# flo-stilz/Audio-Key-Estimation

Measured on AMD Instinct MI355X. Metric: clips/s (15 s @ 22.05 kHz), HIP CQT + PitchClassNet forward, higher is better.
Workload: dtype f32 accumulation everywhere; pitch / semitone / layer-0 convolutions: f16 activations x f16 weights (per-channel power-of-two scaled) on MFMA, one product; last layer's pitch-class convolutions and heads: 3-term split-bf16 on MFMA (hi*hi + lo*hi + hi*lo); CQT filter bank: 3-term split-bf16 on MFMA

## Files before the change

### audio-key-estimation_amd/csrc/pcnet.hip

```cpp
#include <algorithm>
#include <cmath>
#include <cstdlib>
#include <cstring>
#include <map>
#include <string>
#include <vector>

#include "common.h"
#include "pcnet_kernels.h"
#include "pcnet_bwd_kernels.h"

using namespace ake_k;

namespace {

constexpr double kBnEps = 1e-5;
constexpr size_t kLdsBudget = 64 * 1024;
constexpr size_t kBfFragsPerConv = 14 * 2 * 64 + 64;

struct TensorSpec {
    std::string name;
    int64_t shape[4];
    int ndim;
};
// ... 1699 lines not shown
}

int upload_i32(const std::vector<int32_t>& v, int32_t** dev) {
    if (*dev) { (void)hipFree(*dev); *dev = nullptr; }
    AKE_HIP_CHECK(hipMalloc(dev, std::max<size_t>(v.size(), 1) * sizeof(int32_t)));
    AKE_HIP_CHECK(hipMemcpy(*dev, v.data(), v.size() * sizeof(int32_t), hipMemcpyHostToDevice));
    return AKE_OK;
}

int rebuild_dense_affine(ake_pcnet* n, const float* params_dev, hipStream_t s) {
    if (n->aff_recs.empty()) return AKE_OK;
    const int rows = static_cast<int>(n->dense_aff_floats / 3);
    if (!n->dense_aff_dev) {
        std::vector<int32_t> idx;
        idx.reserve(static_cast<size_t>(rows) * 5);
        auto off = [&](const std::string& key) { return static_cast<int32_t>(n->grad_off[n->spec_index.at(key)]); };
        for (const auto& r : n->aff_recs)
            for (int ch = 0; ch < r.C; ++ch) {
                int32_t bits;
                std::memcpy(&bits, &r.slope, sizeof(bits));
                for (const char* f : {".weight", ".bias", ".running_mean", ".running_var"}) idx.push_back(off(r.bn + f) + ch);
                idx.push_back(bits);
            }
        int rc = upload_i32(idx, &n->dense_aff_idx_dev);
        if (rc) return rc;
        AKE_HIP_CHECK(hipMalloc(&n->dense_aff_dev, n->dense_aff_floats * sizeof(float)));
    }
    ake::ProfScope ps("dense_affine_kernel", s);
    hipLaunchKernelGGL(dense_affine_kernel, dim3((rows + 255) / 256), dim3(256), 0, s, params_dev, n->dense_aff_idx_dev, n->dense_aff_dev, rows);
    AKE_HIP_CHECK(hipGetLastError());
    return AKE_OK;
}

int build_fold_tables(ake_pcnet* n) {
    std::vector<int32_t> fold_ch(n->grad_floats, -1), fold_bn, run_off(static_cast<size_t>(n->bn_channels) * 2, 0), run_off2(static_cast<size_t>(n->bn_channels) * 2, -1);
    n->recomputed_bn_channels = 0;
    auto off = [&](const std::string& key) { return static_cast<int32_t>(n->grad_off[n->spec_index.at(key)]); };
    int base = 0;
    for (const auto& r : n->fold_records) {
        const int32_t w0 = off(r.wkey), b0 = off(r.bkey);
        const size_t total = r.per_out * r.cout, k = r.transposed ? r.per_out / r.cin : 0;
        for (size_t i = 0; i < total; ++i) {
            const int co = r.transposed ? static_cast<int>((i / k) % r.cout) : static_cast<int>(i / r.per_out);
            fold_ch[w0 + i] = (base + co) << 1;
        }
        for (int co = 0; co < r.cout; ++co) {
            fold_ch[b0 + co] = ((base + co) << 1) | 1;
            fold_bn.push_back(off(r.bn + ".weight") + co);
            fold_bn.push_back(off(r.bn + ".bias") + co);
            fold_bn.push_back(off(r.bn + ".running_mean") + co);
            fold_bn.push_back(off(r.bn + ".running_var") + co);
        }
        base += r.cout;
    }
    for (const auto& l : n->bns)
        for (int c = 0; c < l.C; ++c) {
            run_off[2 * (l.ch_off + c)] = off(l.name + ".running_mean") + c;
            run_off[2 * (l.ch_off + c) + 1] = off(l.name + ".running_var") + c;
            const bool again = n->cfg.denseblock && l.name.size() > 6 && l.name.compare(l.name.size() - 6, 6, ".norm1") == 0;
            if (again) {
                run_off2[2 * (l.ch_off + c)] = run_off[2 * (l.ch_off + c)];
                run_off2[2 * (l.ch_off + c) + 1] = run_off[2 * (l.ch_off + c) + 1];
                ++n->recomputed_bn_channels;
            }
        }
    int rc;
    if ((rc = upload_i32(fold_ch, &n->fold_ch_dev)) || (rc = upload_i32(fold_bn, &n->fold_bn_dev)) || (rc = upload_i32(run_off, &n->run_off_dev)) || (rc = upload_i32(run_off2, &n->run_off2_dev)) ||
        (rc = upload_i32(n->map_host, &n->map_dev)))
        return rc;
    if (n->folded_dev) { (void)hipFree(n->folded_dev); n->folded_dev = nullptr; }
    AKE_HIP_CHECK(hipMalloc(&n->folded_dev, n->grad_floats * sizeof(float)));
    return AKE_OK;
}

bool pc_bf16_eligible(const PackedConv& pc) { return (pc.kh == 12 || pc.kh == 1) && pc.kw == 7 && pc.cin <= 16 && (pc.cout == 16 || pc.cout == 32); }

int rebuild_bf16_frags(ake_pcnet* n, hipStream_t s, bool train_only = false) {
    size_t count = 0;
    for (auto& layer : n->p2p)
        for (size_t j = 0; j < layer.size(); ++j) {
            PackedConv& pc = layer[j];
            pc.bf_off = -1;
            if (pc.cin <= 8 && pc.cout == 8 && pc.kh == 7 && pc.kw == 7 && pc.co == 8) { pc.bf_off = static_cast<long long>(count); count += kBfFragsPerConv; }
        }
    struct TrainFrag { PackedConv* pc; size_t raw; int cin, cout, flip; };
    std::vector<TrainFrag> tfr;
    if (!n->raw_w_off.empty())
        for (size_t i = 1; i < n->p2p_t.size() && i < n->p2p_d.size(); ++i)
            for (size_t j = 0; j < n->p2p_t[i].size() && j < n->p2p_d[i].size(); ++j) {
                PackedConv& pt = n->p2p_t[i][j];
                PackedConv& pd = n->p2p_d[i][j];
                pt.bf_off = pd.bf_off = -1;
                const auto it = n->spec_index.find("model." + std::to_string(i) + ".p2p.layer." + std::to_string(3 * j) + ".weight");
                if (it == n->spec_index.end() || pt.kh != 7 || pt.kw != 7 || pt.cin > 8 || pt.cout > 8 || n->cfg.resblock || n->cfg.denseblock) continue;
                const size_t raw = n->raw_w_off[it->second];
                pt.bf_off = static_cast<long long>(count); count += kBfFragsPerConv;
                tfr.push_back({&pt, raw, pt.cin, pt.cout, 0});
                pd.bf_off = static_cast<long long>(count); count += kBfFragsPerConv;
                tfr.push_back({&pd, raw, pt.cin, pt.cout, 1});
            }
    std::vector<PackedConv*> tpc;
    if (!n->raw_w_off.empty() && !n->cfg.resblock && !n->cfg.denseblock) {
        for (size_t i = 1; i < n->pc2pc_t.size(); ++i)
            for (PackedConv& pc : n->pc2pc_t[i]) tpc.push_back(&pc);
        if (!n->head_key_t.empty()) tpc.push_back(&n->head_key_t[0]);
        if (!n->head_tonic_t.empty()) tpc.push_back(&n->head_tonic_t[0]);
        if (n->head_genre_t.size() == 2) tpc.push_back(&n->head_genre_t[0]);
    }
    for (PackedConv* pc : tpc) {
        pc->bf_off = -1;
        if (pc_bf16_eligible(*pc)) { pc->bf_off = static_cast<long long>(count); count += static_cast<size_t>(pc->kh) * 4 * (pc->cout / 16) * 2 * 64 + 64; }
    }
    std::vector<PackedConv*> tpd;
    if (!n->raw_w_off.empty() && !n->cfg.resblock && !n->cfg.denseblock)
        for (size_t i = 1; i < n->pc2pc_d.size(); ++i)
            for (PackedConv& pc : n->pc2pc_d[i]) tpd.push_back(&pc);
    for (PackedConv* pc : tpd) {
        pc->bf_off = -1;
        if (pc->kh == 12 && pc->kw == 7 && pc->cin == 16 && pc->cout <= 32) {
            pc->bf_off = static_cast<long long>(count);
            count += static_cast<size_t>(pc->kh) * 4 * ((pc->cout + 15) / 16) * 2 * 64 + 64;
        }
    }
    std::vector<PackedConv*> thd;
    if (!n->raw_w_off.empty() && !n->cfg.resblock && !n->cfg.denseblock && n->cfg.head_layers == 2) {
        if (!n->head_key_d.empty()) thd.push_back(&n->head_key_d[0]);
        if (!n->head_tonic_d.empty()) thd.push_back(&n->head_tonic_d[0]);
        if (!n->head_genre_d.empty()) thd.push_back(&n->head_genre_d[0]);
    }
    for (PackedConv* pc : thd) {
        pc->bf_off = pc->bf_off2 = -1;
        if ((pc->kh == 12 || pc->kh == 1) && pc->kw == 7 && pc->cin == 32 && pc->cout == 16) {
            const size_t one = static_cast<size_t>(pc->kh) * 4 * 2 * 64 + 64;
            pc->bf_off = static_cast<long long>(count); pc->bf_off2 = static_cast<long long>(count + one);
            count += 2 * one;
        }
    }
    std::vector<PackedConv*> pcs;
    for (auto& layer : n->pc2pc)
        for (PackedConv& pc : layer) pcs.push_back(&pc);
    if (!n->head_key.empty()) pcs.push_back(&n->head_key[0]);
    if (!n->head_tonic.empty()) pcs.push_back(&n->head_tonic[0]);
    if (n->head_genre.size() == 2) pcs.push_back(&n->head_genre[0]);
    for (PackedConv* pc : pcs) {
        pc->bf_off = -1;
        if (pc_bf16_eligible(*pc)) { pc->bf_off = static_cast<long long>(count); count += static_cast<size_t>(pc->kh) * 4 * (pc->cout / 16) * 2 * 64; }
    }
    std::vector<PackedConv*> h1;
    if (n->head_key.size() == 2) h1.push_back(&n->head_key[1]);
    if (n->head_tonic.size() == 2) h1.push_back(&n->head_tonic[1]);
    if (n->head_genre.size() == 2) h1.push_back(&n->head_genre[1]);
    for (PackedConv* pc : h1) {
        pc->bf_off = -1;
        if ((pc->kh == 12 || pc->kh == 2) && pc->kw == 7 && pc->cout == 1 && pc->co == 1 && pc->cin == 32) { pc->bf_off = static_cast<long long>(count); count += static_cast<size_t>(pc->kh) * 22 * 2 * 64; }
    }
    if (!n->pc2pc.empty())
        for (PackedConv& pc : n->pc2pc[0]) {
            pc.l0_off = -1;
            if (n->cfg.num_layers > 1 && pc.kh == 12 && pc.kw == 7 && pc.co == 4 && pc.groups == 1 && pc.cout <= 4 && pc.cin <= 4) {
                pc.l0_off = static_cast<long long>(count); count += 24 * 64 + 64;
            }
        }
    for (size_t i = 1; i < n->semi.size(); ++i) {
        PackedConv& pc = n->semi[i];
        pc.bf_off = -1;
        if (pc.cin == 8 && pc.co == 8 && pc.groups == 1 && i < n->p2p.size() && !n->p2p[i].empty() && n->p2p[i].back().bf_off >= 0) {
            pc.bf_off = static_cast<long long>(count); count += 6 * 64 + 64;
        }
    }
    if (count == 0) return AKE_OK;
    if (n->bf_frags_count != count) {
        if (n->bf_frags_dev) { (void)hipFree(n->bf_frags_dev); n->bf_frags_dev = nullptr; }
        AKE_HIP_CHECK(hipMalloc(&n->bf_frags_dev, count * sizeof(uint4)));
        n->bf_frags_count = count;
    }
    ake::ProfScope ps("pack_bf16_kernels", s);
    n->eval_frags_stale = train_only;
    if (!train_only)
    for (const auto& layer : n->p2p)
        for (const PackedConv& pc : layer)
            if (pc.bf_off >= 0)
                hipLaunchKernelGGL(pack_p2p_f16_kernel, dim3((14 * 64 + 255) / 256), dim3(256), 0, s, n->blob_dev + pc.w_off, n->bf_frags_dev + pc.bf_off, pc.cin);
    if (!train_only)
    for (const PackedConv* pc : pcs)
        if (pc->bf_off >= 0) {
            const int NT = pc->cout / 16;
            hipLaunchKernelGGL(pack_pc_bf16_kernel, dim3((pc->kh * 4 * NT * 64 + 255) / 256), dim3(256), 0, s, n->blob_dev + pc->w_off,
                               n->bf_frags_dev + pc->bf_off, pc->cin, pc->cout, pc->co, NT, pc->kh);
        }
    if (!train_only && !n->pc2pc.empty())
        for (const PackedConv& pc : n->pc2pc[0])
            if (pc.l0_off >= 0)
                hipLaunchKernelGGL(pack_l0_f16_kernel, dim3(3), dim3(256), 0, s, n->blob_dev + pc.w_off, n->bf_frags_dev + pc.l0_off, pc.cin, pc.cout);
    {
        std::vector<PcPackJob> jobs;
        auto add = [&](const PackedConv* pc, long long off, int NT, int dy_rot, int ci_off) {
            jobs.push_back(PcPackJob{n->blob_dev + pc->w_off, n->bf_frags_dev + off, pc->cin, pc->cout, pc->co, NT, pc->kh, dy_rot, ci_off});
        };
        for (const PackedConv* pc : tpc)
            if (pc->bf_off >= 0) add(pc, pc->bf_off, pc->cout / 16, 0, 0);
        for (const PackedConv* pc : tpd)
            if (pc->bf_off >= 0) add(pc, pc->bf_off, (pc->cout + 15) / 16, pc->kh - 1, 0);
        for (const PackedConv* pc : thd)
            if (pc->bf_off >= 0)
                for (int half = 0; half < 2; ++half) add(pc, half ? pc->bf_off2 : pc->bf_off, 1, pc->kh - 1, 16 * half);
        for (size_t j0 = 0; j0 < jobs.size(); j0 += kMaxPackJobs) {
            PcPackJobs js;
            js.n = static_cast<int>(std::min<size_t>(kMaxPackJobs, jobs.size() - j0));
            int max_cout = 1, max_blocks = 1;
            for (int k = 0; k < js.n; ++k) {
                js.j[k] = jobs[j0 + k];
                max_cout = std::max(max_cout, js.j[k].cout);
                max_blocks = std::max(max_blocks, (js.j[k].KH * 4 * js.j[k].NT * 64 + 255) / 256);
            }
            hipLaunchKernelGGL(pc_weight_scale_jobs_kernel, dim3(max_cout, js.n), dim3(256), 0, s, js);
            hipLaunchKernelGGL(pack_pc_f16x3_jobs_kernel, dim3(max_blocks, js.n), dim3(256), 0, s, js);
        }
        for (size_t j0 = 0; j0 < tfr.size(); j0 += kMaxPackJobs) {
            P2pRawJobs js;
            js.n = static_cast<int>(std::min<size_t>(kMaxPackJobs, tfr.size() - j0));
            for (int k = 0; k < js.n; ++k) {
                const TrainFrag& t = tfr[j0 + k];
                js.j[k] = P2pRawJob{n->blob_dev + t.raw, n->bf_frags_dev + t.pc->bf_off, t.cin, t.cout, t.flip};
            }
            hipLaunchKernelGGL(pack_p2p_f16_raw_jobs_kernel, dim3((14 * 64 + 255) / 256, js.n), dim3(256), 0, s, js);
        }
    }
    for (size_t i = 1; !train_only && i < n->semi.size(); ++i)
        if (n->semi[i].bf_off >= 0)
            hipLaunchKernelGGL(pack_semi_f16_kernel, dim3(1), dim3(192), 0, s, n->blob_dev + n->semi[i].w_off, n->bf_frags_dev + n->semi[i].bf_off);
    if (!train_only)
    for (const PackedConv* pc : h1)
        if (pc->bf_off >= 0)
            hipLaunchKernelGGL(pack_head1_bf16_kernel, dim3((pc->kh * 22 * 64 + 255) / 256), dim3(256), 0, s, n->blob_dev + pc->w_off,
                               n->bf_frags_dev + pc->bf_off, pc->cin, pc->kh);
    AKE_HIP_CHECK(hipGetLastError());
    return AKE_OK;
}

}

int ake_pcnet_finalize(ake_pcnet* n) {
    AKE_REQUIRE(n, AKE_ERR_INVALID, "finalize: null handle");
    for (size_t i = 0; i < n->specs.size(); ++i)
        AKE_REQUIRE(n->host[i].set, AKE_ERR_STATE, "finalize: missing key '%s' (load_state_dict strict=True)", n->specs[i].name.c_str());
    int rc;
    if (n->map_host.empty()) {
        if ((rc = trace_maps(n))) return rc;
        if ((rc = build_fold_tables(n))) return rc;
    }
    reset_packs(n);
    build_packs(n, false);
    build_packs(n, true);
    n->blob.resize(ake::align_up(n->blob.size() + 64, 64), 0.f);
    AKE_REQUIRE(n->blob.size() == n->map_host.size(), AKE_ERR_STATE, "finalize: blob layout changed between builds");
    if (!n->blob_dev) AKE_HIP_CHECK(hipMalloc(&n->blob_dev, n->blob.size() * sizeof(float)));
    AKE_HIP_CHECK(hipMemcpy(n->blob_dev, n->blob.data(), n->blob.size() * sizeof(float), hipMemcpyHostToDevice));
    if ((rc = rebuild_bf16_frags(n, nullptr))) return rc;
    if (!n->aff_recs.empty()) {
        std::vector<float> flat(n->grad_floats);
        for (size_t i = 0; i < n->specs.size(); ++i) std::copy(n->host[i].data.begin(), n->host[i].data.end(), flat.begin() + n->grad_off[i]);
        float* tmp = nullptr;
        AKE_HIP_CHECK(hipMalloc(&tmp, flat.size() * sizeof(float)));
        AKE_HIP_CHECK(hipMemcpy(tmp, flat.data(), flat.size() * sizeof(float), hipMemcpyHostToDevice));
        rc = rebuild_dense_affine(n, tmp, nullptr);
        AKE_HIP_CHECK(hipStreamSynchronize(nullptr));
        (void)hipFree(tmp);
        if (rc) return rc;
    }
    AKE_HIP_CHECK(hipStreamSynchronize(nullptr));
    n->finalized = true;
    return AKE_OK;
}

namespace {
int load_from_device_impl(ake_pcnet* n, const float* params_dev, ake_stream_t stream, bool train_only);
}
int ake_pcnet_load_from_device_f32(ake_pcnet* n, const float* params_dev, ake_stream_t stream) { return load_from_device_impl(n, params_dev, stream, false); }
int ake_pcnet_load_for_training_f32(ake_pcnet* n, const float* params_dev, ake_stream_t stream) { return load_from_device_impl(n, params_dev, stream, true); }
namespace {
int load_from_device_impl(ake_pcnet* n, const float* params_dev, ake_stream_t stream, bool train_only) {
    AKE_REQUIRE(n && params_dev, AKE_ERR_INVALID, "load_from_device: null argument");
    if (n->map_host.empty()) {
        for (size_t i = 0; i < n->specs.size(); ++i) {
            size_t cnt = 1;
            for (int d = 0; d < n->specs[i].ndim; ++d) cnt *= static_cast<size_t>(n->specs[i].shape[d]);
            if (n->host[i].data.size() != cnt) n->host[i].data.assign(cnt, 0.f);
        }
        int rc;
        if ((rc = trace_maps(n))) return rc;
        if ((rc = build_fold_tables(n))) return rc;
        if (!n->blob_dev) AKE_HIP_CHECK(hipMalloc(&n->blob_dev, n->blob.size() * sizeof(float)));
    }
    hipStream_t s = static_cast<hipStream_t>(stream);
    const int P = static_cast<int>(n->grad_floats), NB = static_cast<int>(n->map_host.size());
    {
        ake::ProfScope ps("fold_params_kernel", s);
        hipLaunchKernelGGL(fold_params_kernel, dim3((P + 255) / 256), dim3(256), 0, s, params_dev, n->fold_ch_dev, n->fold_bn_dev, n->folded_dev, P);
    }
    {
        ake::ProfScope ps("gather_blob_kernel", s);
        hipLaunchKernelGGL(gather_blob_kernel, dim3((NB + 255) / 256), dim3(256), 0, s, params_dev, n->folded_dev, n->map_dev, n->blob_dev, NB);
    }
    AKE_HIP_CHECK(hipGetLastError());
    {
        int rc2 = rebuild_bf16_frags(n, s, train_only);
        if (!rc2) rc2 = rebuild_dense_affine(n, params_dev, s);
        if (rc2) return rc2;
    }
    n->finalized = true;
    return AKE_OK;
}
}

int ake_pcnet_update_running_stats_f32(const ake_pcnet* n, const float* bn_stats_dev, float* params_dev, float momentum, ake_stream_t stream) {
    AKE_REQUIRE(n && bn_stats_dev && params_dev, AKE_ERR_INVALID, "update_running_stats: null argument");
    AKE_REQUIRE(n->finalized && n->run_off_dev, AKE_ERR_STATE, "update_running_stats: the handle has no parameters yet");
    hipStream_t s = static_cast<hipStream_t>(stream);
    ake::ProfScope ps("running_stats_kernel", s);
    hipLaunchKernelGGL(running_stats_kernel, dim3((n->bn_channels + 63) / 64), dim3(64), 0, s, bn_stats_dev, n->run_off_dev, params_dev, momentum,
                       n->bn_channels);
    AKE_HIP_CHECK(hipGetLastError());
    return AKE_OK;
}

int ake_pcnet_update_recomputed_running_stats_f32(const ake_pcnet* n, const float* bn_stats_dev, float* params_dev, float momentum, int* channels,
                                                  ake_stream_t stream) {
    AKE_REQUIRE(n, AKE_ERR_INVALID, "update_recomputed_running_stats: null handle");
    if (channels) *channels = n->recomputed_bn_channels;
    if (n->recomputed_bn_channels == 0) return AKE_OK;
    AKE_REQUIRE(bn_stats_dev && params_dev, AKE_ERR_INVALID, "update_recomputed_running_stats: null argument");
    AKE_REQUIRE(n->finalized && n->run_off2_dev, AKE_ERR_STATE, "update_recomputed_running_stats: the handle has no parameters yet");
    hipStream_t s = static_cast<hipStream_t>(stream);
    ake::ProfScope ps("running_stats_kernel", s);
    hipLaunchKernelGGL(running_stats_kernel, dim3((n->bn_channels + 63) / 64), dim3(64), 0, s, bn_stats_dev, n->run_off2_dev, params_dev, momentum,
                       n->bn_channels);
    AKE_HIP_CHECK(hipGetLastError());
    return AKE_OK;
}

int ake_pcnet_num_bn(const ake_pcnet* n) { return n ? static_cast<int>(n->bns.size()) : 0; }

int ake_pcnet_bn_info(const ake_pcnet* n, int index, const char** name, int* channels, int* channel_offset) {
    AKE_REQUIRE(n && index >= 0 && index < static_cast<int>(n->bns.size()), AKE_ERR_INVALID, "bn_info: index out of range (finalize first)");
    if (name) *name = n->bns[index].name.c_str();
    if (channels) *channels = n->bns[index].C;
    if (channel_offset) *channel_offset = n->bns[index].ch_off;
    return AKE_OK;
}

size_t ake_pcnet_workspace_bytes(const ake_pcnet* n, int batch, int frames) {
    if (!n || batch <= 0 || frames <= 0) return 0;
    Buffers b;
    if (plan_buffers(n, batch, std::min(batch, n->chunk_clips), frames, nullptr, &b) != AKE_OK) return 0;
    return b.bytes;
}

size_t ake_pcnet_train_workspace_bytes(const ake_pcnet* n, int batch, int frames) {
    if (!n || batch <= 0 || frames <= 0) return 0;
    Buffers b;
    if (plan_buffers(n, batch, batch, frames, nullptr, &b, true) != AKE_OK) return 0;
    return b.bytes;
}

namespace {

struct Fwd {
    const ake_pcnet* n;
    Buffers& b;
    hipStream_t s;
    bool train;
    const Route& r;

    int bn_of(const std::string& name) const { return n->bn_index.at(name); }
    float* p2pin_up(int i) const { return train ? b.aff_p2pin[i] + 3 * n->dims[i].prev_p : nullptr; }

    void finalize_bn(int bn, double count, float* aff_out, float slope = kSlope) {
        const auto& l = n->bns[bn];
        ake::ProfScope ps("bn_finalize_kernel", s);
        hipLaunchKernelGGL(bn_finalize_kernel, dim3((l.C + 63) / 64), dim3(64), 0, s, b.stats + 2 * l.ch_off, 2 * n->bn_channels, count,
                           n->blob_dev + l.gamma_off, n->blob_dev + l.beta_off, aff_out, b.bstats + 3 * l.ch_off, l.C, slope);
    }
    void identity(float* aff, int C) {
        hipLaunchKernelGGL(affine_identity_kernel, dim3((C + 63) / 64), dim3(64), 0, s, aff, C);
    }

    int conv(const PackedConv& pe, const PackedConv& pt, const std::string& bn_name, int kind, Src src, const float* in_aff,
// ... 960 lines not shown
```

### audio-key-estimation_amd/csrc/pcnet_kernels.h

```cpp
#pragma once

#include <hip/hip_runtime.h>

#include "common.h"

namespace ake_k {

constexpr int TW = 4;
constexpr float kSlope = 0.01f;

struct ConvArgs {
    const float* src0;
    const float* src1;
    long long src0_clip_stride, src1_clip_stride;
    int c0, c1, h1;
    int H;
    int T_in;
    int T_out;
    int H_out;
    int py;
    int pad_l;
    int time_circ;
    const float* w;
    const float* bias;
// ... 1509 lines not shown
    {
        const float* src = a.src + clip * a.src_clip_stride;
        for (int i = threadIdx.x; i < 12 * T * 2; i += 1024) {
            const int half = i & 1, pos = i >> 1;
            const int y = pos / T, t = pos - y * T;
            unsigned int hi[4] = {0, 0, 0, 0}, lo[4] = {0, 0, 0, 0};
#pragma unroll
            for (int k = 0; k < 8; ++k) {
                const int c = half * 8 + k;
                const float v = c < a.cin ? src[(static_cast<long long>(c) * 12 + y) * T + t] : 0.f;
                const unsigned int hb = bf16_bits(v);
                hi[k >> 1] |= hb << (16 * (k & 1));
                lo[k >> 1] |= bf16_bits(v - __uint_as_float(hb << 16)) << (16 * (k & 1));
            }
            const int idx = ((y * Tp + t + 3) << 1) + half;
            map0[idx] = make_uint4(hi[0], hi[1], hi[2], hi[3]);
            map0[n16 + idx] = make_uint4(lo[0], lo[1], lo[2], lo[3]);
        }
    }
    __syncthreads();
    const int n_tt = (T + 15) >> 4;
    const bool active = wave < 3 * n_tt;
    const int tt = wave / 3, y0 = 4 * (wave - 3 * tt);
    const int t0 = 16 * tt;
    const int dxq = q >> 1, half = q & 1;
    const int lane_off = ((t0 + r16 + dxq) << 1) + half;
    const int lane_off3 = ((t0 + r16 + 6) << 1) + half;
    auto frag_off = [&](int s, int p) {
        int row = y0 + s + (p == 3 ? dxq : 0);
        row -= row >= 12 ? 12 : 0;
        return ((row * Tp) << 1) + (p == 3 ? lane_off3 : lane_off + 4 * p);
    };
    const int Tf = T / 2;
    float* const pooled_c = a.pooled + static_cast<long long>(clip) * 16 * 12 * Tf;
    unsigned short* const fh_c = a.fh ? a.fh + static_cast<long long>(clip) * 12 * Tf * 16 : nullptr;
    unsigned short* const fl_c = a.fh ? a.fl + static_cast<long long>(clip) * 12 * Tf * 16 : nullptr;
    for (int j = 0; j < a.n_conv; ++j) {
        const uint4* const pH = (j & 1) ? map1 : map0;
        const uint4* const pL = pH + n16;
        unsigned short* const oH = reinterpret_cast<unsigned short*>((j & 1) ? map0 : map1);
        unsigned short* const oL = oH + n16 * 8;
        const bool last = j == a.n_conv - 1;
        const uint4* const bfrag_j = j == 0 ? a.bfrag[0] : (j == 1 ? a.bfrag[1] : (j == 2 ? a.bfrag[2] : a.bfrag[3]));
        const float* const bias_j = j == 0 ? a.bias[0] : (j == 1 ? a.bias[1] : (j == 2 ? a.bias[2] : a.bias[3]));
        const uint4* const bfrag_n = j == 0 ? a.bfrag[1] : (j == 1 ? a.bfrag[2] : a.bfrag[3]);
        {
            f32x4c acc[MT];
#pragma unroll
            for (int mt = 0; mt < MT; ++mt) acc[mt] = f32x4c{0.f, 0.f, 0.f, 0.f};
            bf16x8c fh[4], fl[4];
            int c = 0;
            auto run_p = [&](auto pair_c, const int p) __attribute__((always_inline)) {
                constexpr bool PAIR = decltype(pair_c)::value;
                if (active) {
#pragma unroll
                    for (int s = 0; s < 4; ++s) {
                        const int off = frag_off(s, PAIR ? 3 : p);
                        fh[s] = __builtin_bit_cast(bf16x8c, pH[off]);
                        fl[s] = __builtin_bit_cast(bf16x8c, pL[off]);
                    }
                }
#pragma unroll 1
                for (int dq = 0; dq < 3; ++dq, ++c) {
                    uint4 wpre = make_uint4(0, 0, 0, 0);
                    const bool fetch = threadIdx.x < kRow && (c + 1 < 12 || j + 1 < a.n_conv);
                    if (fetch) wpre = c + 1 < 12 ? bfrag_j[dq < 2 ? wsrc(p, dq + 1) : wsrc(p + 1, 0)] : bfrag_n[wsrc(0, 0)];
                    const uint4* const wr = wring + (c & 1) * kRow + lane;
                    if (active) {
#pragma unroll
                        for (int i = 0; i < 4; i += PAIR ? 2 : 1) {
                            const bf16x8c bh = __builtin_bit_cast(bf16x8c, wr[(i * 2 + 0) * 64]), bl = __builtin_bit_cast(bf16x8c, wr[(i * 2 + 1) * 64]);
#pragma unroll
                            for (int mt = 0; mt < MT; ++mt) acc[mt] = __builtin_amdgcn_mfma_f32_16x16x32_bf16(fh[(mt + i) & 3], bh, acc[mt], 0, 0, 0);
#pragma unroll
                            for (int mt = 0; mt < MT; ++mt) acc[mt] = __builtin_amdgcn_mfma_f32_16x16x32_bf16(fl[(mt + i) & 3], bh, acc[mt], 0, 0, 0);
#pragma unroll
                            for (int mt = 0; mt < MT; ++mt) acc[mt] = __builtin_amdgcn_mfma_f32_16x16x32_bf16(fh[(mt + i) & 3], bl, acc[mt], 0, 0, 0);
#pragma unroll
                            for (int u = 0; u < (PAIR ? 2 : 1); ++u) {
                                const int s_new = 4 * dq + i + 4 + u;
                                if (s_new < 12 + MT - (PAIR ? 2 : 1)) {
                                    const int off = frag_off(s_new, PAIR ? 3 : p);
                                    fh[i + u] = __builtin_bit_cast(bf16x8c, pH[off]);
                                    fl[i + u] = __builtin_bit_cast(bf16x8c, pL[off]);
                                }
                            }
                        }
                    }
                    if (fetch) wring[((c + 1) & 1) * kRow + threadIdx.x] = wpre;
                    if (c + 1 < 12) __syncthreads();
                }
            };
#pragma unroll 1
            for (int p = 0; p < 3; ++p) run_p(std::false_type{}, p);
            run_p(std::true_type{}, 3);
            if (active) {
            const int co = r16;
            const float bias = bias_j[co];
            const int tq0 = t0 + 4 * q;
            if (tq0 < T) {
#pragma unroll
            for (int mt = 0; mt < MT; ++mt) {
                    const int y = y0 + mt;
                    float v[4];
#pragma unroll
                    for (int i = 0; i < 4; ++i) {
                        const float x = acc[mt][i] + bias;
                        v[i] = x > 0.f ? x : x * kSlope;
                    }
                    if (!last) {
#pragma unroll
                        for (int i = 0; i < 4; ++i) {
                            const int e = ((((y * Tp + tq0 + i + 3) << 1) + (co >> 3)) << 3) + (co & 7);
                            const unsigned int hb = bf16_bits(v[i]);
                            oH[e] = static_cast<unsigned short>(hb);
                            oL[e] = static_cast<unsigned short>(bf16_bits(v[i] - __uint_as_float(hb << 16)));
                        }
                    } else {
#pragma unroll
                        for (int i = 0; i < 4; i += 2) {
                            const float pv = fmaxf(v[i], v[i + 1]);
                            const int tq = (tq0 + i) >> 1;
                            pooled_c[(co * 12 + y) * Tf + tq] = pv;
                            if (a.fh) {
                                const int e = (y * Tf + tq) * 16 + co;
                                const unsigned int hb = bf16_bits(pv);
                                fh_c[e] = static_cast<unsigned short>(hb);
                                fl_c[e] = static_cast<unsigned short>(bf16_bits(pv - __uint_as_float(hb << 16)));
                            }
                        }
                    }
            }
            }
            }
        }
        __syncthreads();
    }
}

struct Head1BfArgs {
    const unsigned short* xh[3];
    const unsigned short* xl[3];
    const uint4* bfrag[3];
    const float* bias[3];
    float* dst[3];
    int KH[3], H_out[3], circular[3];
    int T_in, T_out, Tp, JB;
    float* pout[3];
    PoolArgs pool;
    int fin_off;
};

constexpr int kHead1MT = 4;
constexpr int kHead1PF = 3;

__device__ __forceinline__ void head1_prefetch(const uint4* __restrict__ bg, int nks, int wave, uint4 (&nbh)[kHead1PF], uint4 (&nbl)[kHead1PF]) {
#pragma unroll
    for (int i = 0; i < kHead1PF; ++i) {
        const int kn = wave + 8 * i < nks ? wave + 8 * i : wave;
        nbh[i] = bg[(2 * kn + 0) * 64]; nbl[i] = bg[(2 * kn + 1) * 64];
    }
}

__device__ __forceinline__ void head1_multiply_store(const uint4* __restrict__ bg, int nks, uint4 (&nbh)[kHead1PF], uint4 (&nbl)[kHead1PF], uint4* lds4,
                                                     int Tp, int HO, int circ, int JB, int T_out, int clip, const float* bias_p, float* dst,
                                                     bool keep, int fin_off) {
    constexpr int PF = kHead1PF;
    const int lane = threadIdx.x & 63;
    const int wave = __builtin_amdgcn_readfirstlane(threadIdx.x >> 6);
    const int r16 = lane & 15, q = lane >> 4;
    const uint4* const pH = lds4;
    const uint4* const pL = lds4 + 12 * Tp * 4;
    float* const red = reinterpret_cast<float*>(lds4);
    const int Mtot = HO * JB;
    const int mtiles = (Mtot + 15) / 16;
    int ay[kHead1MT], af[kHead1MT];
#pragma unroll
    for (int mt = 0; mt < kHead1MT; ++mt) {
        int m = mt * 16 + r16;
        if (m >= Mtot) m = Mtot - 1;
        const int jb = m / HO;
        ay[mt] = m - jb * HO;
        af[mt] = 16 * jb;
    }
    f32x4c acc[kHead1MT];
#pragma unroll
    for (int mt = 0; mt < kHead1MT; ++mt) acc[mt] = f32x4c{0.f, 0.f, 0.f, 0.f};
    for (int ks = wave; ks < nks; ks += 8) {
        const int dy = ks / 22, dxe = ks - dy * 22;
        const bf16x8c bh = __builtin_bit_cast(bf16x8c, nbh[0]);
        const bf16x8c bl = __builtin_bit_cast(bf16x8c, nbl[0]);
#pragma unroll
        for (int i = 0; i + 1 < PF; ++i) { nbh[i] = nbh[i + 1]; nbl[i] = nbl[i + 1]; }
        {
            const int kn = ks + 8 * PF < nks ? ks + 8 * PF : ks;
            nbh[PF - 1] = bg[(2 * kn + 0) * 64]; nbl[PF - 1] = bg[(2 * kn + 1) * 64];
        }
#pragma unroll
        for (int mt = 0; mt < kHead1MT; ++mt) {
            if (mt < mtiles) {
                int row = ay[mt] + dy;
                row -= (circ && row >= 12) ? 12 : 0;
                const int ad = ((row * Tp + af[mt] + dxe) << 2) + q;
                const bf16x8c ah = __builtin_bit_cast(bf16x8c, pH[ad]);
                const bf16x8c al = __builtin_bit_cast(bf16x8c, pL[ad]);
                acc[mt] = __builtin_amdgcn_mfma_f32_16x16x32_bf16(ah, bh, acc[mt], 0, 0, 0);
                acc[mt] = __builtin_amdgcn_mfma_f32_16x16x32_bf16(al, bh, acc[mt], 0, 0, 0);
                acc[mt] = __builtin_amdgcn_mfma_f32_16x16x32_bf16(ah, bl, acc[mt], 0, 0, 0);
            }
        }
    }
    __syncthreads();
#pragma unroll
    for (int mt = 0; mt < kHead1MT; ++mt)
#pragma unroll
        for (int i = 0; i < 4; ++i) red[((wave * kHead1MT + mt) * 4 + i) * 64 + lane] = acc[mt][i];
    __syncthreads();
    if (wave < mtiles) {
        const float bias = bias_p[0];
#pragma unroll
        for (int i = 0; i < 4; ++i) {
            float v = bias;
#pragma unroll
            for (int w = 0; w < 8; ++w) v += red[((w * kHead1MT + wave) * 4 + i) * 64 + lane];
            const int m = wave * 16 + 4 * q + i;
            const int jb = m / HO, y = m - jb * HO;
            const int t = 16 * jb + r16;
            if (m < Mtot && t < T_out) {
                dst[(static_cast<long long>(clip) * HO + y) * T_out + t] = v;
                if (keep) red[fin_off + y * T_out + t] = v;
            }
        }
    }
}

__global__ __launch_bounds__(512) void conv_head1_bf16_kernel(Head1BfArgs a) {
    extern __shared__ __attribute__((aligned(16))) uint4 lds4[];
    const int clip = blockIdx.x, head = blockIdx.y;
    const int lane = threadIdx.x & 63;
    const int wave = __builtin_amdgcn_readfirstlane(threadIdx.x >> 6);
    const int Tp = a.Tp;
    uint4* const pH = lds4;
    uint4* const pL = lds4 + 12 * Tp * 4;
    {
        const long long cbase = static_cast<long long>(clip) * 12 * a.T_in * 4;
        const uint4* gh = reinterpret_cast<const uint4*>(a.xh[head]) + cbase;
        const uint4* gl = reinterpret_cast<const uint4*>(a.xl[head]) + cbase;
        const int n16 = 12 * Tp * 4;
        for (int i = threadIdx.x; i < n16; i += blockDim.x) {
            const int grp = i & 3, pos = i >> 2;
            const int row = pos / Tp, f = pos - row * Tp;
            uint4 vh = make_uint4(0, 0, 0, 0), vl = make_uint4(0, 0, 0, 0);
            if (f < a.T_in) {
                const long long g = (static_cast<long long>(row) * a.T_in + f) * 4 + grp;
                vh = gh[g]; vl = gl[g];
            }
            pH[i] = vh; pL[i] = vl;
        }
    }
    __syncthreads();
    const int HO = a.H_out[head], nks = a.KH[head] * 22;
    const uint4* __restrict__ bg = a.bfrag[head] + lane;
    uint4 nbh[kHead1PF], nbl[kHead1PF];
    head1_prefetch(bg, nks, wave, nbh, nbl);
    head1_multiply_store(bg, nks, nbh, nbl, lds4, Tp, HO, a.circular[head], a.JB, a.T_out, clip, a.bias[head], a.dst[head], a.pout[head] != nullptr,
                         a.fin_off);
    if (a.pout[head] == nullptr) return;
    __syncthreads();
    if (threadIdx.x < HO)
        a.pout[head][clip * HO + threadIdx.x] =
            pool_row(a.pool, reinterpret_cast<const float*>(lds4) + a.fin_off + threadIdx.x * a.T_out, clip, a.T_out, head);
}

struct HeadsFusedArgs {
    const unsigned short* xh;
    const unsigned short* xl;
    const uint4* bfragA[3];
    const float* biasA[3];
    const uint4* bfragB[3];
    const float* biasB[3];
    float* dst[3];
    float* pout[3];
    int KHA[3], KHB[3];
    int hs[3];
    int batch;
    int T_in, T1, T2;
    int TpA, TpB, JB;
    PoolArgs pool;
    int fin_off;
};

template <int MT>
__global__ __launch_bounds__(512, 4) void heads_fused_kernel(HeadsFusedArgs a) {
    extern __shared__ __attribute__((aligned(16))) uint4 lds4[];
#define AKE_HSEL(f) (head == 0 ? a.f[0] : head == 1 ? a.f[1] : a.f[2])
    const int bid = __builtin_amdgcn_readfirstlane(blockIdx.x);
    const int seg = (bid >= a.batch ? 1 : 0) + (bid >= 2 * a.batch ? 1 : 0);
    const int clip = bid - seg * a.batch;
    const int head = seg == 0 ? a.hs[0] : seg == 1 ? a.hs[1] : a.hs[2];
    const int lane = threadIdx.x & 63;
    const int wave = __builtin_amdgcn_readfirstlane(threadIdx.x >> 6);
    const int r16 = lane & 15, q = lane >> 4;
    constexpr int NT = 2;
    const int TpB = a.TpB;
    uint4* const pHB = lds4;
    uint4* const pLB = lds4 + 12 * TpB * 4;
    const uint4* __restrict__ bg = AKE_HSEL(bfragB) + lane;
    const int KHB = AKE_HSEL(KHB);
    const int nks = KHB * 22;
    uint4 nbh[kHead1PF], nbl[kHead1PF];
    {
        const int Mtot = 12 * a.T1;
        const int tile0 = wave * MT;
        const bool active = tile0 * 16 < Mtot;
        f32x4c acc[MT][NT], accl[1][1];
        pc_bf16_multiply<NT, MT, false>(a.xh, a.xl, AKE_HSEL(bfragA), lds4, clip, a.T_in, a.T1, 0, a.TpA, AKE_HSEL(KHA), 8, tile0, Mtot, acc, accl);
        head1_prefetch(bg, nks, wave, nbh, nbl);
        __syncthreads();
        unsigned short* const sH = reinterpret_cast<unsigned short*>(pHB);
        unsigned short* const sL = reinterpret_cast<unsigned short*>(pLB);
        {
            const int nz = TpB - a.T1, n16 = 12 * nz * 4;
            for (int i = threadIdx.x; i < n16; i += 512) {
                const int grp = i & 3, pos = i >> 2;
                const int row = pos / nz, f = a.T1 + pos - row * nz;
                pHB[((row * TpB + f) << 2) + grp] = make_uint4(0, 0, 0, 0);
                pLB[((row * TpB + f) << 2) + grp] = make_uint4(0, 0, 0, 0);
            }
        }
        if (active) {
            const float* const bptr = AKE_HSEL(biasA);
#pragma unroll
            for (int nt = 0; nt < NT; ++nt) {
                const int co = nt * 16 + r16;
                const float bias = bptr[co];
#pragma unroll
                for (int mt = 0; mt < MT; ++mt) {
                    const int m0 = (tile0 + mt) * 16 + 4 * q;
                    int y = m0 / a.T1, t = m0 - y * a.T1;
#pragma unroll
                    for (int i = 0; i < 4; ++i) {
                        if (m0 + i < Mtot) {
                            float v = acc[mt][nt][i] + bias;
                            v = v > 0.f ? v : v * kSlope;
                            const int idx = (y * TpB + t) * 32 + co;
                            const unsigned int hb = bf16_bits(v);
                            sH[idx] = static_cast<unsigned short>(hb);
                            sL[idx] = static_cast<unsigned short>(bf16_bits(v - __uint_as_float(hb << 16)));
                        }
                        if (++t == a.T1) { t = 0; ++y; }
                    }
                }
            }
        }
    }
    __syncthreads();
    const int circ = KHB == 12 ? 1 : 0;
    const int HO = circ ? 12 : 12 - KHB + 1;
    head1_multiply_store(bg, nks, nbh, nbl, lds4, TpB, HO, circ, a.JB, a.T2, clip, AKE_HSEL(biasB), AKE_HSEL(dst), true, a.fin_off);
    __syncthreads();
    if (threadIdx.x < HO)
        AKE_HSEL(pout)[clip * HO + threadIdx.x] = pool_row(a.pool, reinterpret_cast<const float*>(lds4) + a.fin_off + threadIdx.x * a.T2, clip, a.T2, head);
#undef AKE_HSEL
}

__global__ void pack_head1_bf16_kernel(const float* __restrict__ w, uint4* __restrict__ out, int cin, int KH) {
    const int i = blockIdx.x * blockDim.x + threadIdx.x;
    if (i >= KH * 22 * 64) return;
    const int lane = i & 63, ks = i >> 6;
    const int dy = ks / 22, dxe = ks - dy * 22;
    const int tau = lane & 15, qq = lane >> 4;
    const int dx = dxe - tau;
    unsigned int hi[4] = {0, 0, 0, 0}, lo[4] = {0, 0, 0, 0};
    for (int e = 0; e < 8; ++e) {
        const int ci = 8 * qq + e;
        float v = 0.f;
        if (dx >= 0 && dx < 7 && ci < cin) v = w[(ci * KH + dy) * 7 + dx];
        const unsigned int hb = bf16_bits(v);
        hi[e >> 1] |= hb << (16 * (e & 1));
        lo[e >> 1] |= bf16_bits(v - __uint_as_float(hb << 16)) << (16 * (e & 1));
    }
    out[(2 * ks + 0) * 64 + lane] = make_uint4(hi[0], hi[1], hi[2], hi[3]);
    out[(2 * ks + 1) * 64 + lane] = make_uint4(lo[0], lo[1], lo[2], lo[3]);
}

__global__ void pack_pc_bf16_kernel(const float* __restrict__ w, uint4* __restrict__ out, int cin, int cout, int CO, int NT, int KH) {
    const int i = blockIdx.x * blockDim.x + threadIdx.x;
    if (i >= KH * 4 * NT * 64) return;
    const int lane = i & 63, nt = (i >> 6) % NT, ks = i / (64 * NT);
    const int dy = ks >> 2, p = ks & 3;
    const int co = nt * 16 + (lane & 15), qq = lane >> 4;
    const int c8 = 8 * (qq & 1);
    int dx = 2 * p + (qq >> 1), dyw = dy;
    if (p == 3 && !(KH & 1)) {
        dx = (dy & 1) ? 7 : 6;
        dyw = dy + (qq >> 1);
    }
    unsigned int hi[4] = {0, 0, 0, 0}, lo[4] = {0, 0, 0, 0};
    for (int e = 0; e < 8; ++e) {
        const int ci = c8 + e;
        float v = 0.f;
        if (dx < 7 && ci < cin && co < cout) v = w[((((co / CO) * cin + ci) * KH + dyw) * 7 + dx) * CO + (co % CO)];
        const unsigned int hb = bf16_bits(v);
        const unsigned int lb = bf16_bits(v - __uint_as_float(hb << 16));
        hi[e >> 1] |= hb << (16 * (e & 1));
        lo[e >> 1] |= lb << (16 * (e & 1));
    }
    out[((ks * NT + nt) * 2 + 0) * 64 + lane] = make_uint4(hi[0], hi[1], hi[2], hi[3]);
    out[((ks * NT + nt) * 2 + 1) * 64 + lane] = make_uint4(lo[0], lo[1], lo[2], lo[3]);
}

__global__ void nchw_to_cl16_kernel(const float* __restrict__ src, long long src_clip_stride, int C, int T, unsigned short* __restrict__ xh,
                                    unsigned short* __restrict__ xl, long long npos) {
    const long long i = static_cast<long long>(blockIdx.x) * blockDim.x + threadIdx.x;
    if (i >= npos) return;
    const int t = static_cast<int>(i % T);
    const long long r = i / T;
    const int y = static_cast<int>(r % 12);
    const long long clip = r / 12;
    const float* s = src + clip * src_clip_stride + static_cast<long long>(y) * T + t;
    unsigned int hi[8], lo[8];
#pragma unroll
    for (int k = 0; k < 8; ++k) { hi[k] = 0; lo[k] = 0; }
#pragma unroll
    for (int c = 0; c < 16; ++c) {
        const float v = c < C ? s[static_cast<long long>(c) * 12 * T] : 0.f;
        const unsigned int hb = bf16_bits(v);
        hi[c >> 1] |= hb << (16 * (c & 1));
        lo[c >> 1] |= bf16_bits(v - __uint_as_float(hb << 16)) << (16 * (c & 1));
    }
    uint4* oh = reinterpret_cast<uint4*>(xh) + i * 2;
    uint4* ol = reinterpret_cast<uint4*>(xl) + i * 2;
    oh[0] = make_uint4(hi[0], hi[1], hi[2], hi[3]); oh[1] = make_uint4(hi[4], hi[5], hi[6], hi[7]);
    ol[0] = make_uint4(lo[0], lo[1], lo[2], lo[3]); ol[1] = make_uint4(lo[4], lo[5], lo[6], lo[7]);
}

__global__ void nchw_to_cl16_f16x2_kernel(const float* __restrict__ src, long long src_clip_stride, int C, int T, const float* __restrict__ aff,
                                          unsigned short* __restrict__ xh, unsigned short* __restrict__ xl, long long npos,
                                          const unsigned int* __restrict__ amax) {
    const long long i = static_cast<long long>(blockIdx.x) * blockDim.x + threadIdx.x;
    const float mul = amax ? f16_weight_scale(amax_load(amax)) : 1.f;
    if (i >= npos) return;
    const int t = static_cast<int>(i % T);
    const long long r = i / T;
    const int y = static_cast<int>(r % 12);
    const long long clip = r / 12;
    const float* s = src + clip * src_clip_stride + static_cast<long long>(y) * T + t;
    unsigned int hi[8], lo[8];
#pragma unroll
    for (int k = 0; k < 8; ++k) { hi[k] = 0; lo[k] = 0; }
#pragma unroll
    for (int c = 0; c < 16; ++c) {
        float v = 0.f;
        if (c < C) {
            v = s[static_cast<long long>(c) * 12 * T] * mul;
            if (aff) { v = fmaf(v, aff[3 * c], aff[3 * c + 1]); v = v > 0.f ? v : v * aff[3 * c + 2]; }
        }
        const _Float16 h = static_cast<_Float16>(v);
        hi[c >> 1] |= static_cast<unsigned int>(__builtin_bit_cast(unsigned short, h)) << (16 * (c & 1));
        lo[c >> 1] |= f16_bits((v - static_cast<float>(h)) * kP2pLoScale) << (16 * (c & 1));
    }
    uint4* oh = reinterpret_cast<uint4*>(xh) + i * 2;
    uint4* ol = reinterpret_cast<uint4*>(xl) + i * 2;
    oh[0] = make_uint4(hi[0], hi[1], hi[2], hi[3]); oh[1] = make_uint4(hi[4], hi[5], hi[6], hi[7]);
    ol[0] = make_uint4(lo[0], lo[1], lo[2], lo[3]); ol[1] = make_uint4(lo[4], lo[5], lo[6], lo[7]);
}

struct PcPackJob { const float* w; uint4* out; int cin, cout, CO, NT, KH, dy_rot, ci_off; };
constexpr int kMaxPackJobs = 24;
struct PcPackJobs { int n; PcPackJob j[kMaxPackJobs]; };
struct P2pRawJob { const float* w; uint4* out; int cin_fwd, cout_fwd, transpose_flip; };
struct P2pRawJobs { int n; P2pRawJob j[kMaxPackJobs]; };

__device__ __forceinline__ void pc_weight_scale_body(const float* __restrict__ w, float* __restrict__ inv_scale, int cin, int cout, int CO, int KH, int bx) {
    __shared__ float red[4];
    const int co = bx;
    const int g = co / CO, c = co - g * CO;
    float m = 0.f;
    for (int r = threadIdx.x; r < cin * KH * 7; r += blockDim.x) m = fmaxf(m, fabsf(w[(static_cast<long long>(g) * cin * KH * 7 + r) * CO + c]));
#pragma unroll
    for (int o = 32; o > 0; o >>= 1) m = fmaxf(m, __shfl_xor(m, o));
    if ((threadIdx.x & 63) == 0) red[threadIdx.x >> 6] = m;
    __syncthreads();
    if (threadIdx.x == 0) inv_scale[co] = 1.f / f16_weight_scale(fmaxf(fmaxf(red[0], red[1]), fmaxf(red[2], red[3])));
}
__global__ __launch_bounds__(256) void pc_weight_scale_kernel(const float* __restrict__ w, float* __restrict__ inv_scale, int cin, int cout, int CO, int KH) {
    pc_weight_scale_body(w, inv_scale, cin, cout, CO, KH, blockIdx.x);
}
__global__ __launch_bounds__(256) void pc_weight_scale_jobs_kernel(PcPackJobs js) {
    const PcPackJob& J = js.j[blockIdx.y];
    if (static_cast<int>(blockIdx.x) >= J.cout) return;
    pc_weight_scale_body(J.w, reinterpret_cast<float*>(J.out + J.KH * 4 * J.NT * 2 * 64), J.cin, J.cout, J.CO, J.KH, blockIdx.x);
}

__device__ __forceinline__ void pack_pc_f16x3_body(const float* __restrict__ w, uint4* __restrict__ out, int cin, int cout, int CO, int NT, int KH, int dy_rot,
                                                   int ci_off, int bx) {
    const int i = bx * blockDim.x + threadIdx.x;
    if (i >= KH * 4 * NT * 64) return;
    const int lane = i & 63, nt = (i >> 6) % NT, ks = i / (64 * NT);
    const int dy = ks >> 2, p = ks & 3;
    const int co = nt * 16 + (lane & 15), qq = lane >> 4;
    const int c8 = 8 * (qq & 1);
    int dx = 2 * p + (qq >> 1), dyw = dy;
    if (p == 3 && !(KH & 1)) {
        dx = (dy & 1) ? 7 : 6;
        dyw = dy + (qq >> 1);
    }
    const float sc = co < cout ? 1.f / reinterpret_cast<const float*>(out + KH * 4 * NT * 2 * 64)[co] : 1.f;
    unsigned int hi[4] = {0, 0, 0, 0}, lo[4] = {0, 0, 0, 0};
    for (int e = 0; e < 8; ++e) {
        const int ci = ci_off + c8 + e;
        float v = 0.f;
        if (dx < 7 && ci < cin && co < cout) v = sc * w[((((co / CO) * cin + ci) * KH + (dyw + dy_rot) % KH) * 7 + dx) * CO + (co % CO)];
        const _Float16 hv = static_cast<_Float16>(v);
        hi[e >> 1] |= static_cast<unsigned int>(__builtin_bit_cast(unsigned short, hv)) << (16 * (e & 1));
        lo[e >> 1] |= f16_bits((v - static_cast<float>(hv)) * kP2pLoScale) << (16 * (e & 1));
    }
    out[((ks * NT + nt) * 2 + 0) * 64 + lane] = make_uint4(hi[0], hi[1], hi[2], hi[3]);
    out[((ks * NT + nt) * 2 + 1) * 64 + lane] = make_uint4(lo[0], lo[1], lo[2], lo[3]);
}
__global__ void pack_pc_f16x3_jobs_kernel(PcPackJobs js) {
    const PcPackJob& J = js.j[blockIdx.y];
    pack_pc_f16x3_body(J.w, J.out, J.cin, J.cout, J.CO, J.NT, J.KH, J.dy_rot, J.ci_off, blockIdx.x);
}

// ... 894 lines not shown
```

Baseline: 491,800.

## Remap circular head1 conv to pitch-row-as-N MFMA layout with fewer k-steps

For the circular (KH=12) head1 convolution, the weights are now packed so that the MFMA N dimension indexes the 12 output pitch rows (circular shift folded into the weight fragment). This reduces the k-steps from 12*22 to 12*7, and the M tiles now run over time blocks (JB up to 5). A dedicated reduction and store path handles the circular case. The non-circular path drops its wrap logic. The change relies on JB <= 5 and adds a separate code path to maintain.

Result: faster. 502,000, median of 6 (+2.1%).

```diff
diff --git a/audio-key-estimation_amd/csrc/pcnet.hip b/audio-key-estimation_amd/csrc/pcnet.hip
--- a/audio-key-estimation_amd/csrc/pcnet.hip
+++ b/audio-key-estimation_amd/csrc/pcnet.hip
@@ -1875,7 +1875,7 @@
     if (n->head_genre.size() == 2) h1.push_back(&n->head_genre[1]);
     for (PackedConv* pc : h1) {
         pc->bf_off = -1;
-        if ((pc->kh == 12 || pc->kh == 2) && pc->kw == 7 && pc->cout == 1 && pc->co == 1 && pc->cin == 32) { pc->bf_off = static_cast<long long>(count); count += static_cast<size_t>(pc->kh) * 22 * 2 * 64; }
+        if ((pc->kh == 12 || pc->kh == 2) && pc->kw == 7 && pc->cout == 1 && pc->co == 1 && pc->cin == 32) { pc->bf_off = static_cast<long long>(count); count += static_cast<size_t>(head1_ksteps(pc->kh)) * 2 * 64; }
     }
     if (!n->pc2pc.empty())
         for (PackedConv& pc : n->pc2pc[0]) {
@@ -1955,7 +1955,7 @@
     if (!train_only)
     for (const PackedConv* pc : h1)
         if (pc->bf_off >= 0)
-            hipLaunchKernelGGL(pack_head1_bf16_kernel, dim3((pc->kh * 22 * 64 + 255) / 256), dim3(256), 0, s, n->blob_dev + pc->w_off,
+            hipLaunchKernelGGL(pack_head1_bf16_kernel, dim3((head1_ksteps(pc->kh) * 64 + 255) / 256), dim3(256), 0, s, n->blob_dev + pc->w_off,
                                n->bf_frags_dev + pc->bf_off, pc->cin, pc->kh);
     AKE_HIP_CHECK(hipGetLastError());
     return AKE_OK;
diff --git a/audio-key-estimation_amd/csrc/pcnet_kernels.h b/audio-key-estimation_amd/csrc/pcnet_kernels.h
--- a/audio-key-estimation_amd/csrc/pcnet_kernels.h
+++ b/audio-key-estimation_amd/csrc/pcnet_kernels.h
@@ -1685,6 +1685,8 @@
 };
 
 constexpr int kHead1MT = 4;
+constexpr int kHead1JB = 5;
+__host__ __device__ constexpr int head1_ksteps(int KH) { return KH == 12 ? 12 * 7 : KH * 22; }
 constexpr int kHead1PF = 3;
 
 __device__ __forceinline__ void head1_prefetch(const uint4* __restrict__ bg, int nks, int wave, uint4 (&nbh)[kHead1PF], uint4 (&nbl)[kHead1PF]) {
@@ -1705,6 +1707,55 @@
     const uint4* const pH = lds4;
     const uint4* const pL = lds4 + 12 * Tp * 4;
     float* const red = reinterpret_cast<float*>(lds4);
+    if (circ) {
+        f32x4c acc[kHead1JB];
+#pragma unroll
+        for (int mt = 0; mt < kHead1JB; ++mt) acc[mt] = f32x4c{0.f, 0.f, 0.f, 0.f};
+        for (int ks = wave; ks < nks; ks += 8) {
+            const int r = ks / 7, dx = ks - r * 7;
+            const bf16x8c bh = __builtin_bit_cast(bf16x8c, nbh[0]);
+            const bf16x8c bl = __builtin_bit_cast(bf16x8c, nbl[0]);
+#pragma unroll
+            for (int i = 0; i + 1 < PF; ++i) { nbh[i] = nbh[i + 1]; nbl[i] = nbl[i + 1]; }
+            {
+                const int kn = ks + 8 * PF < nks ? ks + 8 * PF : ks;
+                nbh[PF - 1] = bg[(2 * kn + 0) * 64]; nbl[PF - 1] = bg[(2 * kn + 1) * 64];
+            }
+            const int ad0 = ((r * Tp + r16 + dx) << 2) + q;
+#pragma unroll
+            for (int mt = 0; mt < kHead1JB; ++mt) {
+                if (mt < JB) {
+                    const bf16x8c ah = __builtin_bit_cast(bf16x8c, pH[ad0 + 64 * mt]);
+                    const bf16x8c al = __builtin_bit_cast(bf16x8c, pL[ad0 + 64 * mt]);
+                    acc[mt] = __builtin_amdgcn_mfma_f32_16x16x32_bf16(ah, bh, acc[mt], 0, 0, 0);
+                    acc[mt] = __builtin_amdgcn_mfma_f32_16x16x32_bf16(al, bh, acc[mt], 0, 0, 0);
+                    acc[mt] = __builtin_amdgcn_mfma_f32_16x16x32_bf16(ah, bl, acc[mt], 0, 0, 0);
+                }
+            }
+        }
+        __syncthreads();
+#pragma unroll
+        for (int mt = 0; mt < kHead1JB; ++mt)
+            if (mt < JB)
+#pragma unroll
+                for (int i = 0; i < 4; ++i) red[((wave * JB + mt) * 4 + i) * 64 + lane] = acc[mt][i];
+        __syncthreads();
+        if (wave < JB) {
+            const float bias = bias_p[0];
+#pragma unroll
+            for (int i = 0; i < 4; ++i) {
+                float v = bias;
+#pragma unroll
+                for (int w = 0; w < 8; ++w) v += red[((w * JB + wave) * 4 + i) * 64 + lane];
+                const int t = 16 * wave + 4 * q + i;
+                if (r16 < 12 && t < T_out) {
+                    dst[(static_cast<long long>(clip) * 12 + r16) * T_out + t] = v;
+                    if (keep) red[fin_off + r16 * T_out + t] = v;
+                }
+            }
+        }
+        return;
+    }
     const int Mtot = HO * JB;
     const int mtiles = (Mtot + 15) / 16;
     int ay[kHead1MT], af[kHead1MT];
@@ -1732,9 +1783,7 @@
 #pragma unroll
         for (int mt = 0; mt < kHead1MT; ++mt) {
             if (mt < mtiles) {
-                int row = ay[mt] + dy;
-                row -= (circ && row >= 12) ? 12 : 0;
-                const int ad = ((row * Tp + af[mt] + dxe) << 2) + q;
+                const int ad = (((ay[mt] + dy) * Tp + af[mt] + dxe) << 2) + q;
                 const bf16x8c ah = __builtin_bit_cast(bf16x8c, pH[ad]);
                 const bf16x8c al = __builtin_bit_cast(bf16x8c, pL[ad]);
                 acc[mt] = __builtin_amdgcn_mfma_f32_16x16x32_bf16(ah, bh, acc[mt], 0, 0, 0);
@@ -1792,7 +1841,7 @@
         }
     }
     __syncthreads();
-    const int HO = a.H_out[head], nks = a.KH[head] * 22;
+    const int HO = a.H_out[head], nks = head1_ksteps(a.KH[head]);
     const uint4* __restrict__ bg = a.bfrag[head] + lane;
     uint4 nbh[kHead1PF], nbl[kHead1PF];
     head1_prefetch(bg, nks, wave, nbh, nbl);
@@ -1840,7 +1889,7 @@
     uint4* const pLB = lds4 + 12 * TpB * 4;
     const uint4* __restrict__ bg = AKE_HSEL(bfragB) + lane;
     const int KHB = AKE_HSEL(KHB);
-    const int nks = KHB * 22;
+    const int nks = head1_ksteps(KHB);
     uint4 nbh[kHead1PF], nbl[kHead1PF];
     {
         const int Mtot = 12 * a.T1;
@@ -1899,11 +1948,18 @@
 
 __global__ void pack_head1_bf16_kernel(const float* __restrict__ w, uint4* __restrict__ out, int cin, int KH) {
     const int i = blockIdx.x * blockDim.x + threadIdx.x;
-    if (i >= KH * 22 * 64) return;
+    if (i >= head1_ksteps(KH) * 64) return;
     const int lane = i & 63, ks = i >> 6;
-    const int dy = ks / 22, dxe = ks - dy * 22;
-    const int tau = lane & 15, qq = lane >> 4;
-    const int dx = dxe - tau;
+    const int col = lane & 15, qq = lane >> 4;
+    int dy, dx;
+    if (KH == 12) {
+        const int r = ks / 7;
+        dx = col < 12 ? ks - r * 7 : -1;
+        dy = r - col + (r < col ? 12 : 0);
+    } else {
+        dy = ks / 22;
+        dx = ks - dy * 22 - col;
+    }
     unsigned int hi[4] = {0, 0, 0, 0}, lo[4] = {0, 0, 0, 0};
     for (int e = 0; e < 8; ++e) {
         const int ci = 8 * qq + e;
```
